# kdexd/probnmn-clevr

Hardware: AMD Instinct MI355X
Metric: CLEVR questions/sec (joint_training step) (higher is better)
Workload: dtype f32; 1 GPU; joint_training_ours.yml (NMN + seq2seq + REINFORCE), global batch 1024 = 1024 questions per GPU x 1 (BASELINE configs[3]), 14x14x1024 features, half of the batch with program supervision, fwd+bwd+[all-reduce]+clamp+Adam; global_batch=1024, per_gpu_batch=1024, parallelism=dp1

## Files before the change

include/probnmn_hip.h:

```cpp
#ifndef PROBNMN_HIP_H
#define PROBNMN_HIP_H

#include <stdint.h>

#ifdef __cplusplus
extern "C" {
#endif

#define PNMN_EINVAL (-1)
#define PNMN_ESHAPE (-2)

#define PNMN_CHANNELS 128

typedef struct pnmn_conv_item {
    const float* in;
    const float* in2;
    const float* mask;
    const float* gate;
    const float* weight;
    const float* bias;
    float*       out;
    int32_t      dilation;
    int32_t      flags;
    const float* mb_feats;
// ... 356 lines not shown
    const int64_t* tokens;
    int64_t        token_stride;
    const float*   w_hh;
    const float*   w_ih;
    const float*   bias;
    float*         hs;
    float*         cs;
    float*         act;
    const float*   dhs;
    float*         dgates;
    int32_t        B, T, dep, reserved;
} pnmn_lstm_stack_job;
int64_t pnmn_lstm_stack_workspace_bytes(const pnmn_lstm_stack_job* jobs , int n, int backward);
int pnmn_lstm_stack_fwd(const pnmn_lstm_stack_job* jobs , int n, void* workspace, void* stream);
int pnmn_lstm_stack_bwd(const pnmn_lstm_stack_job* jobs , int n, void* workspace, void* stream);

typedef struct pnmn_lstm_dropout_desc {
    float*   hsd;
    uint64_t seed;
    int64_t  row_offset;
    float    p;
    int32_t  reserved;
} pnmn_lstm_dropout_desc;
int pnmn_lstm_dropout(const float* x, float* y, int rows, int T, int H, float p, uint64_t seed, int64_t row_offset, void* stream);
int pnmn_lstm_stack_fwd_dropout(const pnmn_lstm_stack_job* jobs , const pnmn_lstm_dropout_desc* drops , int n,
                                void* workspace, void* stream);
int pnmn_lstm_stack_bwd_dropout(const pnmn_lstm_stack_job* jobs , const pnmn_lstm_dropout_desc* drops , int n,
                                void* workspace, void* stream);

#define PNMN_GEMM_MAX 8
#define PNMN_GEMM_A_TRANSPOSED 1
#define PNMN_GEMM_B_TRANSPOSED 2
#define PNMN_GEMM_ACCUMULATE   4
typedef struct pnmn_gemm_desc {
    const float* a;
    const float* b;
    float*       c;
    const float* bias;
    int64_t      lda, ldb, ldc;
    int32_t      M, N, K;
    int32_t      flags;
    int32_t      split_k;
    int32_t      shift_t;
    const float* shift_h0;
    int64_t      ld_h0;
    float*       workspace;
    float*       colsum;
    float*       colsum2;
} pnmn_gemm_desc;
int pnmn_gemm(const pnmn_gemm_desc* descs , int n, void* stream);
int pnmn_gemm_cus(const pnmn_gemm_desc* descs , int n, int max_workgroups, void* stream);
int64_t pnmn_gemm_workspace_bytes(int M, int N, int split_k);
int pnmn_gemm_split_k(int M, int N, int K, int cus);

int pnmn_colsum(const float* x, int64_t ld, int R, int C, float* out, float* out2, int accumulate, void* workspace, void* stream);
int64_t pnmn_colsum_workspace_bytes(int R, int C);

int pnmn_abi_version(void);

#ifdef __cplusplus
}
#endif
#endif
```

probnmn-clevr_amd/csrc/gemm.hip:

```cpp
#include <hip/hip_runtime.h>
#include <stdint.h>

#include <type_traits>

#include "../../include/probnmn_hip.h"
#include "global_ptr.h"
#include "lds_optin.h"

namespace {

typedef float f32x16 __attribute__((ext_vector_type(16)));
using pnmn::as_global;
using pnmn::gfloat;

constexpr int TM = 128, TN = 128, TK = 32;
constexpr int OP_FLOATS = TM * TK;
using lchar = __attribute__((address_space(3))) char;
using gchar = __attribute__((address_space(1))) char;

struct Batch {
    pnmn_gemm_desc d[PNMN_GEMM_MAX];
    int first[PNMN_GEMM_MAX + 1];
    int n;
};

template <bool KC>
__device__ __forceinline__ void load_tile(const gfloat* base, int64_t ld, int row0, int k0, int rows, int K, bool vec, int tid,
                                          f32x4 (&r)[4], int shift_t, const gfloat* h0, int64_t ld_h0) {
#pragma unroll
    for (int j = 0; j < 4; ++j) {
        const int p = tid + 256 * j;
        f32x4 v = f32x4{0.f, 0.f, 0.f, 0.f};
        if (KC) {
            const int row = row0 + (p >> 3), k = k0 + 4 * (p & 7);
            if (row < rows && k < K) {
                const gfloat* src = base + (int64_t)row * ld + k;
                if (vec && k + 3 < K) {
                    v = pnmn::load4(src);
                } else {
#pragma unroll
                    for (int e = 0; e < 4; ++e)
                        if (k + e < K) v[e] = src[e];
                }
            }
        } else {
            const int k = k0 + (p >> 5), row = row0 + 4 * (p & 31);
            if (k < K && row < rows) {
                const gfloat* src;
                bool zero = false;
                if (shift_t > 0) {
                    const int b = k / shift_t;
// ... 64 lines not shown
    int64_t piece, step;
    uint32_t off;

    __device__ __forceinline__ void start(const gfloat* origin, int64_t ld, int row0, int k0, int tid) {
        const int wave = __builtin_amdgcn_readfirstlane(tid >> 6), lane = tid & 63;
        const uint64_t o64 = (uint64_t)(uintptr_t)origin;
        const gchar* o = (const gchar*)(((uint64_t)(uint32_t)__builtin_amdgcn_readfirstlane((int)(o64 >> 32)) << 32) |
                                        (uint32_t)__builtin_amdgcn_readfirstlane((int)(uint32_t)o64));
        if (KC) {
            const int c = (lane & 7) ^ (lane >> 4);
            base = o + ((int64_t)(row0 + 32 * wave) * ld + k0) * 4;
            v0 = (uint32_t)((lane >> 3) * ld) * 4u + 16u * c, v1 = (uint32_t)((lane >> 3) * ld) * 4u + 16u * (c ^ 4);
            piece = 32 * ld, step = 4 * TK, off = (uint32_t)wave * 32u * 128u;
        } else {
            base = o + ((int64_t)(k0 + 8 * wave) * ld + row0) * 4;
            v0 = v1 = (uint32_t)((lane >> 5) * ld) * 4u + 16u * (lane & 31);
            piece = 8 * ld, step = 4 * (int64_t)TK * ld, off = (uint32_t)wave * 8u * 512u;
        }
    }
    __device__ __forceinline__ void issue(float* tile) {
        const uint32_t dst = __builtin_amdgcn_readfirstlane((uint32_t)(uintptr_t)((lchar*)tile)) + off;
#pragma unroll
        for (int j = 0; j < 4; ++j) {
            const uint64_t src = (uint64_t)(uintptr_t)(base + j * piece);
            asm volatile("s_mov_b32 m0, %2\n\ts_nop 0\n\tglobal_load_lds_dwordx4 %0, %1"
                         :
                         : "v"(KC && (j & 1) ? v1 : v0), "s"(src), "s"(dst + 1024u * j)
                         : "memory");
        }
        base += step;
    }
};

template <bool AKC, bool BKC>
__device__ __forceinline__ void contract(const pnmn_gemm_desc& d, int m0, int n0, int kbeg, int kend, float* lds, f32x16 (&acc)[2][2],
                                         bool want_cs, float (&cs)[2]) {
    const int tid = threadIdx.x, wave = tid >> 6, lane = tid & 63, i = lane & 31, h = lane >> 5;
    const int wm = wave >> 1, wn = wave & 1;
    const gfloat* A = as_global(d.a);
    const gfloat* Bm = as_global(d.b);
    const gfloat* h0 = as_global(d.shift_h0);
    const bool avec = (d.lda & 3) == 0 && ((uintptr_t)d.a & 15) == 0;
    const bool bvec = (d.ldb & 3) == 0 && ((uintptr_t)d.b & 15) == 0 && (d.shift_t == 0 || d.shift_h0 == nullptr ||
                                                                       ((d.ld_h0 & 3) == 0 && ((uintptr_t)d.shift_h0 & 15) == 0));
    float* la = lds;
    float* lb = lds + 2 * OP_FLOATS;
    const bool adir = avec && m0 + TM <= d.M, bdir = bvec && n0 + TN <= d.N && (BKC || d.shift_t == 0);
    const int kfull = kbeg + (kend - kbeg) / TK * TK;
    const float rcp_t = d.shift_t > 0 ? 1.f / (float)d.shift_t : 0.f;
    Direct<AKC> da;
    Direct<BKC> db;
    da.start(A, d.lda, m0, kbeg, tid);
    db.start(Bm, d.ldb, n0, kbeg, tid);
    auto loop = [&](auto ad_tag, auto bd_tag, int lo, int hi) {
        constexpr bool AD = decltype(ad_tag)::value, BD = decltype(bd_tag)::value;
        f32x4 ra[4], rb[4];
        auto fetch = [&](int k0, int st) {
            if constexpr (AD)
                da.issue(la + st * OP_FLOATS);
            else
                load_tile<AKC>(A, d.lda, m0, k0, d.M, kend, avec, tid, ra, 0, nullptr, 0);
            if constexpr (BD)
                db.issue(lb + st * OP_FLOATS);
            else if constexpr (AD && !BKC)
                load_tile_shift(Bm, d.ldb, n0, k0, tid, rb, d.shift_t, rcp_t, h0, d.ld_h0);
            else
                load_tile<BKC>(Bm, d.ldb, n0, k0, d.N, kend, bvec, tid, rb, BKC ? 0 : d.shift_t, h0, d.ld_h0);
        };
        auto commit = [&](int st) {
            if constexpr (!AD) store_tile<AKC>(la + st * OP_FLOATS, tid, ra);
            if constexpr (!BD) store_tile<BKC>(lb + st * OP_FLOATS, tid, rb);
        };
        if (lo >= hi) return;
        fetch(lo, 0);
        commit(0);
        asm volatile("s_waitcnt vmcnt(0)" ::: "memory");
        __syncthreads();
        int cur = 0;
        for (int k0 = lo; k0 < hi; k0 += TK) {
            const bool more = k0 + TK < hi;
            if (more) fetch(k0 + TK, cur ^ 1);
            const float* ca = la + cur * OP_FLOATS;
            const float* cb = lb + cur * OP_FLOATS;
#pragma unroll
            for (int q = 0; q < 4; ++q) {
                f32x4 a[2], b[2];
#pragma unroll
                for (int t = 0; t < 2; ++t) {
                    a[t] = frag<AKC>(ca, 64 * wm + 32 * t + i, q, h);
                    b[t] = frag<BKC>(cb, 64 * wn + 32 * t + i, q, h);
                }
                if (!AKC && want_cs) {
#pragma unroll
                    for (int t = 0; t < 2; ++t) cs[t] += (a[t][0] + a[t][1]) + (a[t][2] + a[t][3]);
                }
#pragma unroll
                for (int s = 0; s < 4; ++s)
#pragma unroll
                    for (int mt = 0; mt < 2; ++mt)
#pragma unroll
                        for (int nt = 0; nt < 2; ++nt)
                            acc[mt][nt] = __builtin_amdgcn_mfma_f32_32x32x2f32(a[mt][s], b[nt][s], acc[mt][nt], 0, 0, 0);
            }
            if (more) commit(cur ^ 1);
            asm volatile("s_waitcnt vmcnt(0)" ::: "memory");
            __syncthreads();
            cur ^= 1;
        }
    };
    using yes = std::true_type;
    using no = std::false_type;
    if (adir && bdir) {
        loop(yes{}, yes{}, kbeg, kfull);
        loop(no{}, no{}, kfull, kend);
    } else if (!BKC && adir && bvec && d.shift_t > 0 && n0 + TN <= d.N && kend <= (1 << 21)) {
        if constexpr (!BKC) {
            loop(yes{}, no{}, kbeg, kfull);
            loop(no{}, no{}, kfull, kend);
        }
    } else {
        loop(no{}, no{}, kbeg, kend);
    }
}

__global__ __launch_bounds__(256) __attribute__((amdgpu_waves_per_eu(2, 2))) void gemm_kernel(const Batch batch) {
    extern __shared__ __attribute__((aligned(16))) float lds[];
    for (int unit = blockIdx.x; unit < batch.first[batch.n]; unit += gridDim.x) {
    int pi = 0;
    while (pi + 1 < batch.n && unit >= batch.first[pi + 1]) ++pi;
    const pnmn_gemm_desc d = batch.d[pi];
    const int local = unit - batch.first[pi];
    const int tiles_n = (d.N + TN - 1) / TN, tiles_m = (d.M + TM - 1) / TM;
    const int split = d.split_k > 1 ? d.split_k : 1;
    const int chunk = local % split, tile = local / split;
    const int tm = tile / tiles_n, tn = tile % tiles_n;
    const int m0 = tm * TM, n0 = tn * TN;
    const int ktiles = (d.K + TK - 1) / TK;
    const int per = ktiles / split, extra = ktiles % split;
    const int kt0 = chunk * per + (chunk < extra ? chunk : extra);
    const int kt1 = kt0 + per + (chunk < extra ? 1 : 0);
    const int kbeg = kt0 * TK, kend = kt1 * TK < d.K ? kt1 * TK : d.K;

    f32x16 acc[2][2];
#pragma unroll
    for (int mt = 0; mt < 2; ++mt)
#pragma unroll
        for (int nt = 0; nt < 2; ++nt)
#pragma unroll
            for (int r = 0; r < 16; ++r) acc[mt][nt][r] = 0.f;
    const bool akc = !(d.flags & PNMN_GEMM_A_TRANSPOSED), bkc = (d.flags & PNMN_GEMM_B_TRANSPOSED) != 0;
    const bool want_cs = d.colsum != nullptr && !akc && tn == 0 && ((threadIdx.x >> 6) & 1) == 0;
    const bool tile_cs = d.colsum != nullptr && !akc && tn == 0;
    float cs[2] = {0.f, 0.f};
    if (kbeg < kend) {
        if (akc && bkc)
            contract<true, true>(d, m0, n0, kbeg, kend, lds, acc, false, cs);
        else if (akc)
            contract<true, false>(d, m0, n0, kbeg, kend, lds, acc, false, cs);
        else if (bkc)
            contract<false, true>(d, m0, n0, kbeg, kend, lds, acc, want_cs, cs);
        else
            contract<false, false>(d, m0, n0, kbeg, kend, lds, acc, want_cs, cs);
    }

    int tid = threadIdx.x, m0e = m0, n0e = n0;
    asm volatile("" : "+v"(tid), "+s"(m0e), "+s"(n0e));
    const int wave = tid >> 6, lane = tid & 63, i = lane & 31, h = lane >> 5;
    const int wm = wave >> 1, wn = wave & 1;
    if (tile_cs) {
        if (want_cs) {
#pragma unroll
            for (int t = 0; t < 2; ++t) lds[h * TM + 64 * wm + 32 * t + i] = cs[t];
        }
        __syncthreads();
        if (tid < TM) {
            const float t = lds[tid] + lds[TM + tid];
            if (split > 1) {
                as_global(d.workspace)[(size_t)tiles_m * tiles_n * split * (TM * TN) + ((size_t)tm * split + chunk) * TM + tid] = t;
            } else if (m0e + tid < d.M) {
                d.colsum[m0e + tid] = t;
                if (d.colsum2) d.colsum2[m0e + tid] = t;
            }
        }
        __syncthreads();
    }
    if (split > 1) {
        gfloat* ws = as_global(d.workspace) + ((size_t)tile * split + chunk) * (TM * TN);
#pragma unroll
        for (int mt = 0; mt < 2; ++mt)
#pragma unroll
            for (int nt = 0; nt < 2; ++nt)
#pragma unroll
                for (int r = 0; r < 16; ++r)
                    ws[(64 * wm + 32 * mt + 8 * (r >> 2) + 4 * h + (r & 3)) * TN + 64 * wn + 32 * nt + i] = acc[mt][nt][r];
        continue;
    }
    gfloat* C = as_global(d.c);
    const gfloat* bias = as_global(d.bias);
    const bool accumulate = (d.flags & PNMN_GEMM_ACCUMULATE) != 0;
#pragma unroll
    for (int nt = 0; nt < 2; ++nt) {
        const int col = n0e + 64 * wn + 32 * nt + i;
        if (col >= d.N) continue;
        const float bv = d.bias ? bias[col] : 0.f;
#pragma unroll
        for (int mt = 0; mt < 2; ++mt)
#pragma unroll
            for (int r = 0; r < 16; ++r) {
                const int row = m0e + 64 * wm + 32 * mt + 8 * (r >> 2) + 4 * h + (r & 3);
                if (row < d.M) {
                    gfloat* dst = C + (int64_t)row * d.ldc + col;
                    float v = acc[mt][nt][r] + bv;
                    if (accumulate) v += *dst;
                    *dst = v;
                }
            }
    }
    }
}

__global__ __launch_bounds__(256) void gemm_reduce_kernel(const Batch batch) {
    int pi = 0;
    while (pi + 1 < batch.n && (int)blockIdx.x >= batch.first[pi + 1]) ++pi;
    const pnmn_gemm_desc d = batch.d[pi];
    const int local = blockIdx.x - batch.first[pi];
    const int tiles_n = (d.N + TN - 1) / TN;
    const int quarter = local & 3, tile = local >> 2;
    const int m0 = (tile / tiles_n) * TM + 32 * quarter, n0 = (tile % tiles_n) * TN;
    const int split = d.split_k, tid = threadIdx.x;
    const gfloat* wt = as_global(d.workspace) + (size_t)tile * split * (TM * TN) + quarter * (32 * TN);
    f32x4 sum[4];
#pragma unroll
    for (int j = 0; j < 4; ++j) sum[j] = f32x4{0.f, 0.f, 0.f, 0.f};
    for (int c = 0; c < split; ++c) {
        const gfloat* wc = wt + (size_t)c * (TM * TN);
        f32x4 v[4];
#pragma unroll
        for (int j = 0; j < 4; ++j) v[j] = pnmn::load4(wc + 4 * (tid + 256 * j));
#pragma unroll
        for (int j = 0; j < 4; ++j) sum[j] += v[j];
    }
    if (d.colsum && (d.flags & PNMN_GEMM_A_TRANSPOSED) && quarter == 0 && tile % tiles_n == 0 && tid < TM) {
        const int tiles_m = (d.M + TM - 1) / TM, tm = tile / tiles_n;
        const gfloat* wc = as_global(d.workspace) + (size_t)tiles_m * tiles_n * split * (TM * TN) + (size_t)tm * split * TM + tid;
        float t = 0.f;
        for (int c = 0; c < split; ++c) t += wc[(size_t)c * TM];
        if (tm * TM + tid < d.M) {
            d.colsum[tm * TM + tid] = t;
            if (d.colsum2) d.colsum2[tm * TM + tid] = t;
        }
    }
    gfloat* C = as_global(d.c);
    const gfloat* bias = as_global(d.bias);
    const bool accumulate = (d.flags & PNMN_GEMM_ACCUMULATE) != 0;
    const bool cvec = (d.ldc & 3) == 0 && ((uintptr_t)d.c & 15) == 0;
#pragma unroll
    for (int j = 0; j < 4; ++j) {
        const int p = tid + 256 * j, row = m0 + (p >> 5), col = n0 + 4 * (p & 31);
        if (row >= d.M || col >= d.N) continue;
        gfloat* dst = C + (int64_t)row * d.ldc + col;
        f32x4 v = sum[j];
        if (cvec && col + 3 < d.N) {
            if (d.bias) {
// ... 53 lines not shown
        last_flag = old == slices - 1;
        if (last_flag) counter[blockIdx.x] = 0;
    }
    __syncthreads();
    if (!last_flag || c >= C) return;
    __threadfence();
    float total = 0.f;
    for (int k = 0; k < slices; ++k) total += __builtin_nontemporal_load(partial + (size_t)k * C + c);
    if (accumulate) total += out[c];
    out[c] = total;
    if (out2) out2[c] = total;
}

}

extern "C" int64_t pnmn_gemm_workspace_bytes(int M, int N, int split_k) {
    if (split_k <= 1) return 0;
    const int64_t tiles_m = (M + TM - 1) / TM, tiles = tiles_m * ((N + TN - 1) / TN);
    return (tiles * split_k * (TM * TN) + tiles_m * split_k * TM) * (int64_t)sizeof(float);
}

extern "C" int pnmn_gemm_split_k(int M, int N, int K, int cus) {
    const int64_t tiles = (int64_t)((M + TM - 1) / TM) * ((N + TN - 1) / TN);
    const int ktiles = (K + TK - 1) / TK;
    if (cus <= 0) cus = 256;
    int64_t want = (2 * (int64_t)cus + tiles - 1) / tiles;
    if (tiles >= cus) want = 1;
    const int most = ktiles / 4 > 0 ? ktiles / 4 : 1;
    if (want > most) want = most;
    if (want > 64) want = 64;
    return want < 1 ? 1 : (int)want;
}

extern "C" int pnmn_gemm(const pnmn_gemm_desc* descs, int n, void* stream) { return pnmn_gemm_cus(descs, n, 0, stream); }

extern "C" int pnmn_gemm_cus(const pnmn_gemm_desc* descs, int n, int max_workgroups, void* stream) {
    if (n <= 0) return 0;
    if (!descs || n > PNMN_GEMM_MAX) return PNMN_EINVAL;
    Batch b;
    int blocks = 0, live = 0;
    for (int k = 0; k < n; ++k) {
        const pnmn_gemm_desc& d = descs[k];
        if (d.M <= 0 || d.N <= 0) continue;
        if (!d.a || !d.b || !d.c || d.K < 0) return PNMN_EINVAL;
        if (d.split_k > 1 && !d.workspace) return PNMN_EINVAL;
        if (d.shift_t > 0 && (d.flags & PNMN_GEMM_B_TRANSPOSED)) return PNMN_ESHAPE;
        if (d.colsum && !(d.flags & PNMN_GEMM_A_TRANSPOSED)) return PNMN_ESHAPE;
        b.d[live] = d;
        b.first[live] = blocks;
        const int tiles = ((d.M + TM - 1) / TM) * ((d.N + TN - 1) / TN);
        blocks += tiles * (d.split_k > 1 ? d.split_k : 1);
        ++live;
    }
    if (!live) return 0;
    b.first[live] = blocks;
    b.n = live;
    constexpr size_t lds = (size_t)4 * OP_FLOATS * sizeof(float);
    static std::atomic<uint64_t> cfg{0};
    if (const int e = pnmn::opt_in_lds(reinterpret_cast<const void*>(gemm_kernel), lds, cfg)) return e;
    const int grid = (max_workgroups > 0 && max_workgroups < blocks) ? max_workgroups : blocks;
    hipLaunchKernelGGL(gemm_kernel, dim3(grid), dim3(256), lds, static_cast<hipStream_t>(stream), b);
    Batch r;
    int rblocks = 0, rlive = 0;
    for (int k = 0; k < live; ++k) {
        if (b.d[k].split_k <= 1) continue;
        r.d[rlive] = b.d[k];
        r.first[rlive] = rblocks;
        rblocks += 4 * ((b.d[k].M + TM - 1) / TM) * ((b.d[k].N + TN - 1) / TN);
        ++rlive;
    }
    if (rlive) {
        r.first[rlive] = rblocks;
        r.n = rlive;
        hipLaunchKernelGGL(gemm_reduce_kernel, dim3(rblocks), dim3(256), 0, static_cast<hipStream_t>(stream), r);
    }
    return (int)hipGetLastError();
}

extern "C" int64_t pnmn_colsum_workspace_bytes(int R, int C) {
    (void)R;
    return (int64_t)128 * C * sizeof(float) + (int64_t)((C + 255) / 256) * sizeof(int);
}

extern "C" int pnmn_colsum(const float* x, int64_t ld, int R, int C, float* out, float* out2, int accumulate, void* workspace,
                           void* stream) {
    if (C <= 0) return 0;
    if (!out || !workspace || (R > 0 && !x)) return PNMN_EINVAL;
    int slices = (R + 63) / 64;
    if (slices > 128) slices = 128;
    if (slices < 1) slices = 1;
    float* partial = static_cast<float*>(workspace);
    int* counter = reinterpret_cast<int*>(partial + (size_t)128 * C);
    const int vec = (ld & 3) == 0 && ((uintptr_t)x & 15) == 0;
    hipLaunchKernelGGL(colsum_kernel, dim3((C + 255) / 256, slices), dim3(256), 0, static_cast<hipStream_t>(stream), x, ld, R, C,
                       partial, counter, out, out2, accumulate, vec);
    return (int)hipGetLastError();
}
```

probnmn-clevr_amd/probnmn/_hip.py:

```python
import ctypes
import os
import time
from typing import Dict, Optional

import numpy as np
import torch

_HERE = os.path.dirname(os.path.abspath(__file__))
LIB_PATH = os.environ.get("PNMN_LIB") or os.path.join(os.path.dirname(_HERE), "lib", "libprobnmn_hip.so")

CHANNELS = 128
CONV_ACCUMULATE = 1
CONV_ATOMIC = 2
CONV_MASKBWD = 4
CONV_DATTN = 16


class HipLibraryError(RuntimeError):
    pass


_lib: Optional[ctypes.CDLL] = None

_P = ctypes.c_void_p
# ... 51 lines not shown
    "pnmn_attn_lstm_fwd": (_P,) * 15 + (_I,) * 9 + (ctypes.c_uint64, ctypes.c_uint64, _P, ctypes.c_int64, _P),
    "pnmn_attn_lstm_bwd": (_P,) * 14 + (_I,) * 4 + (_P,),
    "pnmn_attn_lstm_group_workspace_bytes": (_P, _I, _I),
    "pnmn_attn_lstm_fwd_group": (_P, _I, _I, _P, _P),
    "pnmn_attn_lstm_bwd_group": (_P, _I, _I, _P, _P),
    "pnmn_attn_denc": (_P, _P, _P, _P, _P, _P, _I, _I, _I, _I, _P),
    "pnmn_conv_nhwc_launches": (_I, _I, _I, _I, _I, _I),
    "pnmn_conv_force_split": (_I,),
    "pnmn_run_launches": (_P, _I, _P),
    "pnmn_conv2d_nhwc": (_P, _P),
    "pnmn_conv2d_weight_floats": (_I, _I, _I, _I),
    "pnmn_maxpool3x3s2_nhwc": (_P, _P, _I, _I, _I, _I, _P),
    "pnmn_launch_trace_begin": (),
    "pnmn_launch_trace_end": (_P, _I, _P),
    "pnmn_set_rows": (_P, _I, _P),
    "pnmn_trunk_planner_create": (_P, _P),
    "pnmn_trunk_planner_destroy": (_P,),
    "pnmn_trunk_plan_and_launch": (_P, _P, _P),
    "pnmn_trunk_last_forward": (_P, _P, _I),
    "pnmn_trunk_last_records_bytes": (_P, _P, ctypes.c_int64),
    "pnmn_plan_batch": (_P, _P, ctypes.c_int64, _P, _P, _I),
    "pnmn_compile_programs": (_P, _I, _I, _P, _I, _I, _P, _P, _P, _P),
    "pnmn_sample_tokens": (_P, _P, _P, _I, _I, _I, ctypes.c_uint64, ctypes.c_uint64, ctypes.c_uint32, _I, _I, _I, _P),
    "pnmn_lstm_stack_workspace_bytes": (_P, _I, _I),
    "pnmn_lstm_stack_fwd": (_P, _I, _P, _P),
    "pnmn_lstm_stack_bwd": (_P, _I, _P, _P),
    "pnmn_lstm_dropout": (_P, _P, _I, _I, _I, _F, ctypes.c_uint64, ctypes.c_int64, _P),
    "pnmn_lstm_stack_fwd_dropout": (_P, _P, _I, _P, _P),
    "pnmn_lstm_stack_bwd_dropout": (_P, _P, _I, _P, _P),
    "pnmn_gemm": (_P, _I, _P),
    "pnmn_gemm_cus": (_P, _I, _I, _P),
    "pnmn_gemm_workspace_bytes": (_I, _I, _I),
    "pnmn_gemm_split_k": (_I, _I, _I, _I),
    "pnmn_colsum": (_P, ctypes.c_int64, _I, _I, _P, _P, _I, _P, _P),
    "pnmn_colsum_workspace_bytes": (_I, _I),
}


ABI_VERSION = 13


def lib() -> ctypes.CDLL:
    global _lib
    if _lib is None:
        if not os.path.exists(LIB_PATH):
            raise HipLibraryError(
                "libprobnmn_hip.so not found at %s -- build it with `python -c 'import "
                "__graft_entry__ as g; g.build()'` (hipcc --offload-arch=gfx950); there is no "
                "fallback path" % LIB_PATH
            )
        handle = ctypes.CDLL(LIB_PATH)
        for name, argtypes in SIGNATURES.items():
            fn = getattr(handle, name)
            fn.restype = ctypes.c_int64 if name.endswith("_bytes") else ctypes.c_int
            fn.argtypes = list(argtypes)
        if handle.pnmn_abi_version() != ABI_VERSION:
            raise HipLibraryError("%s has ABI version %d, this package binds version %d -- rebuild the library"
                                  % (LIB_PATH, handle.pnmn_abi_version(), ABI_VERSION))
        _lib = handle
    return _lib


_TRACE = None


def check(code: int, what: str) -> None:
# ... 71 lines not shown
     ("a_channels", _i32), ("b_channels", _i32), ("is_max", _i32), ("reserved", _i32)]
)
MASKBWD_ITEM = np.dtype([("dx", _u64), ("feats", _u64), ("attn", _u64), ("dfeats", _u64), ("dattn", _u64)])
AXPY_ITEM = np.dtype([("src", _u64), ("dst", _u64), ("n", np.int64)])
DERIVE_JOB = np.dtype([("src", _u64), ("src2", _u64), ("dst", _u64), ("n", _i32), ("k", _i32), ("ld", _i32), ("kind", _i32)])
PLAN_IN = np.dtype([(n, _u64) for n in ("tables", "nprims", "tids", "examples", "base", "tokens", "w3", "b3", "wt3",
                                         "dotw", "dotb", "params", "grads", "wt", "act", "gact", "feat", "gfeat",
                                         "final_", "gfinal", "ones")]
                   + [(n, _i32) for n in ("n_templates", "pmax", "nv", "cmax", "hw", "channels", "wgrad_chunk",
                                          "wgrad_groups", "fuse_mask_bwd", "sole_writer", "sort_by_weight", "reserved")])
TRUNK_CONFIG = np.dtype([(n, _u64) for n in ("kinds", "w3", "b3", "wt3", "dotw", "dotb")]
                        + [(n, _i32) for n in ("n_kinds", "channels", "H", "W", "wgrad_chunk", "wgrad_groups", "fuse_mask_bwd",
                                               "sole_writer", "sort_by_weight", "reserved")])
TRUNK_IO = np.dtype([(n, _u64) for n in ("programs", "params", "grads", "wt", "act", "gact", "feat", "gfeat", "final_", "gfinal",
                                          "ones")]
                    + [("act_capacity", np.int64)]
                    + [(n, _u64) for n in ("fwd_tail", "bwd_head", "bwd_tail", "bwd", "valid")]
                    + [("arena_floats", np.int64)]
                    + [(n, _i32) for n in ("n_programs", "length", "n_fwd_tail", "n_bwd_head", "n_bwd_tail", "bwd_capacity",
                                           "need_backward", "launch", "n_bwd", "bwd_piece_cut", "n_prims", "n_fwd", "depth",
                                           "n_invalid", "n_feat_result", "conv_cus", "wgrad_cus", "n_conv", "n_proj", "reserved")]
                    + [("touched_tokens", _u64, (4,))])
DECODER_FWD_JOB = np.dtype([(n, _u64) for n in ("xe", "etable", "enc", "mask", "h0", "w_c", "w_hh", "w_p", "b_p", "hs", "cs", "act",
                                                  "ctx", "probs", "tokens", "in_tokens")]
                           + [("in_token_stride", np.int64), ("seed", _u64), ("row_offset", _u64)]
                           + [(n, _i32) for n in ("B", "T", "S", "V", "sample", "pad_index", "unk_index", "start_index")])
DECODER_BWD_JOB = np.dtype([(n, _u64) for n in ("dhs", "act", "cs", "hs", "probs", "enc", "mask", "h0", "w_c_t", "w_hh_t", "dgates",
                                                  "dctx", "dscore", "weights", "dh0")]
                           + [(n, _i32) for n in ("B", "T", "S", "reserved")])
GEMM_DESC = np.dtype([(n, _u64) for n in ("a", "b", "c", "bias")] + [(n, np.int64) for n in ("lda", "ldb", "ldc")]
                     + [(n, _i32) for n in ("M", "N", "K", "flags", "split_k", "shift_t")]
                     + [("shift_h0", _u64), ("ld_h0", np.int64), ("workspace", _u64), ("colsum", _u64), ("colsum2", _u64)])
GEMM_MAX, GEMM_A_T, GEMM_B_T, GEMM_ACC = 8, 1, 2, 4
LSTM_STACK_JOB = np.dtype([("xp", _u64), ("tokens", _u64), ("token_stride", np.int64)] + [(n, _u64) for n in ("w_hh", "w_ih", "bias", "hs", "cs", "act", "dhs", "dgates")]
                          + [(n, _i32) for n in ("B", "T", "dep", "reserved")])
LSTM_STACK_JOBS = 6
LSTM_DROPOUT_DESC = np.dtype([("hsd", _u64), ("seed", _u64), ("row_offset", np.int64), ("p", np.float32), ("reserved", _i32)])
TOKEN_SEG = np.dtype([("src", _u64), ("index", _u64), ("row_stride", np.int64), ("rows", _i32), ("width", _i32)])
EINVAL, ESHAPE, EAGAIN = -1, -2, -3
ADAM_ITEM = np.dtype([("param", _u64), ("grad", _u64), ("exp_avg", _u64), ("exp_avg_sq", _u64), ("n", np.int64),
                      ("bc1", np.float32), ("bc2_sqrt", np.float32)])

LAUNCH = np.dtype([("a", _u64), ("b", _u64), ("c", _u64), ("op", _i32), ("n", _i32), ("p", _i32, (8,))])
CONV2D_DESC = np.dtype([("x", _u64), ("w", _u64), ("scale", _u64), ("shift", _u64), ("residual", _u64), ("y", _u64),
                        ("N", _i32), ("H", _i32), ("W", _i32), ("Cin", _i32), ("Ho", _i32), ("Wo", _i32), ("Cout", _i32),
                        ("kh", _i32), ("kw", _i32), ("stride", _i32), ("pad", _i32), ("relu", _i32)])
LAUNCH_TIMING = np.dtype([("op", _i32), ("n", _i32), ("p", _i32, (8,)), ("n_items", _i32), ("ms", np.float32),
                          ("flops", np.float64), ("bytes", np.float64)])
(OP_CONV, OP_WGRAD, OP_TRANSPOSE_WEIGHTS, OP_DOT_FWD, OP_DOT_BWD, OP_SAME_FWD, OP_SAME_BWD, OP_MINMAX_FWD, OP_MINMAX_BWD,
 OP_MASK_BWD, OP_MAXPOOL_FWD, OP_MAXPOOL_BWD, OP_NCHW_TO_NHWC, OP_SET_ROWS, OP_ACCUMULATE, OP_ZERO, OP_FEAT_GATHER) = range(17)


class LaunchList:

    def __init__(self):
        self._rows = []

    def add(self, op: int, n: int, a: int, b: int = 0, c: int = 0, p=()) -> None:
        q = tuple(p) + (0,) * (8 - len(p))
        self._rows.append((a, b, c, op | (n << 32), q[0] | (q[1] << 32), q[2] | (q[3] << 32), q[4] | (q[5] << 32),
                           q[6] | (q[7] << 32)))

    def __len__(self) -> int:
        return len(self._rows)

    def run(self, stream: int, what: str) -> None:
# ... 135 lines not shown
```

probnmn-clevr_amd/probnmn/runtime/seq_plan.py:

```python
from typing import Dict, List, Optional

import numpy as np
import torch

from probnmn import _hip


SPLIT_SLOTS = int(__import__("os").environ.get("PNMN_PLAN_SPLIT_SLOTS", "512"))
SPLIT_MIN_KTILES = int(__import__("os").environ.get("PNMN_PLAN_SPLIT_MIN", "8"))
USE_STACK = True
import os as _os
STACK_FWD_ENCODERS = int(_os.environ.get("PNMN_PLAN_FWD_ENC", "2"))
STACK_PG_ENCODER = int(_os.environ.get("PNMN_PLAN_PG_ENC", "1"))
STACK_BWD_ENCODERS = int(_os.environ.get("PNMN_PLAN_BWD_ENC", "0"))
DECODER_BWD_GROUP = int(_os.environ.get("PNMN_PLAN_DEC_GROUP", "3"))
GEMM_WORKGROUPS = int(_os.environ.get("PNMN_PLAN_GEMM_WGS", "0"))
USE_AUX_STREAM = _os.environ.get("PNMN_PLAN_AUX", "0") != "0"
_AUX_STREAMS: Dict = {}


def _aux_stream(dev: torch.device) -> "torch.cuda.Stream":
    key = dev.index if dev.index is not None else torch.cuda.current_device()
    if key not in _AUX_STREAMS:
        _AUX_STREAMS[key] = torch.cuda.Stream(device=dev)
    return _AUX_STREAMS[key]


class PlanUnsupported(Exception):
    """The models / shapes are outside what the plan is built for: the trainer keeps the eager passes."""


class _Calls(list):
    def add(self, name: str, *args) -> None:
        self.append((getattr(_hip.lib(), name), args, name))

    def add_fn(self, name: str, fn) -> None:
        self.append((fn, (), name))

    def run(self) -> None:
        for fn, args, name in self:
            rc = fn(*args)
            if rc:
# ... 60 lines not shown
        self.with_prior = with_prior
        B = n + m
        self.B = B
        D = pg._max_decoding_steps
        self.D = D
        if _hip.decoder_workspace_bytes([n, m], False) <= 0 or _hip.decoder_workspace_bytes([B], False) <= 0 \
                or int(lib.pnmn_lstm_seq_workspace_bytes(B, 0)) <= 0:
            raise PlanUnsupported("batch does not fit the multi-CU recurrent kernels in one launch")
        self._bufs: Dict[str, torch.Tensor] = {}
        self._keep: List = []
        self.anchor = torch.zeros((), device=dev, requires_grad=True)
        self.fwd_pg_enc, self.fwd_pg, self.fwd_qr, self.fwd_prior, self.bwd = _Calls(), _Calls(), _Calls(), _Calls(), _Calls()
        self._derived_sig = None
        self._build()

    def buf(self, name: str, *shape, dtype=torch.float32, zero: bool = False) -> torch.Tensor:
        if name in self._bufs:
            raise KeyError(name)
        t = (torch.zeros if zero else torch.empty)(*shape, dtype=dtype, device=self.dev)
        self._bufs[name] = t
        return t

    def bytes_buf(self, name: str, nbytes: int, zero: bool = False) -> torch.Tensor:
        return self.buf(name, max(int(nbytes), 16), dtype=torch.uint8, zero=zero)

    def __getitem__(self, name: str) -> torch.Tensor:
        return self._bufs[name]

    def _gemm(self, calls: _Calls, name: str, descs) -> None:
        lib = _hip.lib()
        for lo in range(0, len(descs), _hip.GEMM_MAX):
            part = descs[lo:lo + _hip.GEMM_MAX]
            rec = np.zeros(len(part), _hip.GEMM_DESC)
            tiles = [((d["M"] + 127) // 128) * ((d["N"] + 127) // 128) for d in part]
            ktiles = [(d["K"] + 31) // 32 for d in part]
            auto = [i for i, d in enumerate(part) if d.get("split") == "auto"]
            fixed_units = sum(t for i, t in enumerate(tiles) if i not in auto)
            chunk_len, best = SPLIT_MIN_KTILES, None
            for cand in range(SPLIT_MIN_KTILES, 129):
                splits = [max(1, min(-(-ktiles[i] // cand), 64)) for i in auto]
                units = fixed_units + sum(tiles[i] * sp for i, sp in zip(auto, splits))
                longest = max([-(-ktiles[i] // sp) for i, sp in zip(auto, splits)] + [ktiles[i] for i in range(len(part)) if i not in auto] + [1])
                rounds = units // SPLIT_SLOTS + (0.6 if units % SPLIT_SLOTS else 0.0)
                cost = rounds * longest + 4.0 * sum(tiles[i] * sp for i, sp in zip(auto, splits) if sp > 1) / SPLIT_SLOTS
                if best is None or cost < best:
                    chunk_len, best = cand, cost
            for i, d in enumerate(part):
                r = rec[i]
                r["a"], r["b"], r["c"] = d["a"], d["b"], d["c"]
                r["lda"], r["ldb"], r["ldc"] = d["lda"], d["ldb"], d["ldc"]
                r["M"], r["N"], r["K"] = d["M"], d["N"], d["K"]
                r["flags"] = (_hip.GEMM_A_T if d.get("ta") else 0) | (_hip.GEMM_B_T if d.get("tb") else 0) | (_hip.GEMM_ACC if d.get("acc") else 0)
                r["bias"] = d.get("bias", 0)
                split = d.get("split", 1)
                if split == "auto":
                    split = max(1, min(-(-ktiles[i] // chunk_len), 64))
                r["split_k"] = split
                if split > 1:
                    ws = self.bytes_buf("%s.ws%d" % (name, lo + i), lib.pnmn_gemm_workspace_bytes(d["M"], d["N"], split), zero=True)
                    r["workspace"] = ws.data_ptr()
                r["shift_t"], r["shift_h0"], r["ld_h0"] = d.get("shift_t", 0), d.get("h0", 0), d.get("ld_h0", 0)
                r["colsum"], r["colsum2"] = d.get("colsum", 0), d.get("colsum2", 0)
            self._keep.append(rec)
            calls.add("pnmn_gemm_cus", rec.ctypes.data, len(rec), GEMM_WORKGROUPS, self.stream)

    def _encoder_prepare(self, calls: _Calls, tag: str, mm: Optional[_Model], derived, tokens: torch.Tensor, width: int, rows: int,
                         drop_first: bool, emb: torch.Tensor, pad_idx, lstm, want_last: bool = True, p: float = 0.0) -> Dict:
        st = self.stream
        model = mm.model if mm is not None else self.prior
        pad, bos, eos = model._pad_index, model._start_index, model._end_index
        T = width + 2 - int(drop_first)
        V = emb.size(0)
        f = self.buf
        e = dict(tag=tag, mm=mm, derived=derived, lstm=lstm, T=T, rows=rows, V=V, pad_idx=-1 if pad_idx is None else pad_idx, emb=emb,
                 want_last=want_last,
                 src=f(tag + ".src", rows, T, dtype=torch.long), fmask=f(tag + ".fmask", rows, T), last=f(tag + ".last", rows, dtype=torch.int32),
                 table=f(tag + ".table", V, 1024), hs1=f(tag + ".hs1", rows, T, 256), cs1=f(tag + ".cs1", rows, T, 256),
                 act1=f(tag + ".act1", rows, T, 1024), hs2=f(tag + ".hs2", rows, T, 256), cs2=f(tag + ".cs2", rows, T, 256),
                 act2=f(tag + ".act2", rows, T, 1024), p=p, seed=0, row_offset=0, drop_recs=[])
        if p > 0:
            e["hsd"] = f(tag + ".hsd", rows, T, 256)
        calls.add("pnmn_token_prep", tokens.data_ptr(), tokens.stride(0), rows, width, pad, bos, eos, int(drop_first), e["src"].data_ptr(),
                  e["fmask"].data_ptr(), e["last"].data_ptr(), st)
        calls.add("pnmn_token_table_fwd", emb.data_ptr(), lstm.weight_ih_l0.data_ptr(), lstm.weight_ih_l0.stride(0),
                  derived["l0.b"].data_ptr(), V, 256, 1024, e["table"].data_ptr(), st)
        if want_last:
            e["enc"], e["h"] = f(tag + ".enc", rows, T, 256), f(tag + ".h", rows, 256)
        return e

    def _stack_jobs(self, encs: List[Dict], backward: bool) -> np.ndarray:
        jobs = np.zeros(2 * len(encs), _hip.LSTM_STACK_JOB)
        for k, e in enumerate(encs):
            d = e["derived"]
            if not backward:
                a, b = jobs[2 * k], jobs[2 * k + 1]
# ... 460 lines not shown
```

Before: 37220 questions/s.

## Move split-K planning to C, add partial-tail splitting and direct shifted B loads

Moves the split-K chunk-length search from Python into a C planner (pnmn_gemm_plan). The planner adds a new mode: when the last GEMM leaves a partial final round of workgroups, only those leftover tiles are split along K while the rest stay whole. This aims to fill the idle slots of the last wave. It also adds a DirectShift loader that streams the time-shifted B operand straight into LDS with global_load_lds, replacing the register-staged path, so shifted LSTM-style GEMMs can use direct LDS loads. The extra encoding in flags and the negative split_k add complexity and reduction overhead, and the cost heuristics may mis-predict.

```diff
diff --git a/include/probnmn_hip.h b/include/probnmn_hip.h
--- a/include/probnmn_hip.h
+++ b/include/probnmn_hip.h
@@ -412,6 +412,9 @@
 #define PNMN_GEMM_A_TRANSPOSED 1
 #define PNMN_GEMM_B_TRANSPOSED 2
 #define PNMN_GEMM_ACCUMULATE   4
+#define PNMN_GEMM_SPLIT_AUTO   8
+#define PNMN_GEMM_SHIFT_REGISTERS 16
+#define PNMN_GEMM_WHOLE_SHIFT  8
 typedef struct pnmn_gemm_desc {
     const float* a;
     const float* b;
@@ -432,6 +435,9 @@
 int pnmn_gemm_cus(const pnmn_gemm_desc* descs , int n, int max_workgroups, void* stream);
 int64_t pnmn_gemm_workspace_bytes(int M, int N, int split_k);
 int pnmn_gemm_split_k(int M, int N, int K, int cus);
+int pnmn_gemm_plan(pnmn_gemm_desc* descs , int n, int cus);
+int64_t pnmn_gemm_plan_workspace_bytes(const pnmn_gemm_desc* desc);
+int pnmn_gemm_plan_units(const pnmn_gemm_desc* desc);
 
 int pnmn_colsum(const float* x, int64_t ld, int R, int C, float* out, float* out2, int accumulate, void* workspace, void* stream);
 int64_t pnmn_colsum_workspace_bytes(int R, int C);
diff --git a/probnmn-clevr_amd/csrc/gemm.hip b/probnmn-clevr_amd/csrc/gemm.hip
--- a/probnmn-clevr_amd/csrc/gemm.hip
+++ b/probnmn-clevr_amd/csrc/gemm.hip
@@ -17,6 +17,16 @@
 constexpr int OP_FLOATS = TM * TK;
 using lchar = __attribute__((address_space(3))) char;
 using gchar = __attribute__((address_space(1))) char;
+
+__host__ __device__ inline int plan_chunks(const pnmn_gemm_desc& d) { return d.split_k > 1 ? d.split_k : d.split_k < -1 ? -d.split_k : 1; }
+__host__ __device__ inline int plan_whole(const pnmn_gemm_desc& d) {
+    return d.split_k < -1 ? (int)((uint32_t)d.flags >> PNMN_GEMM_WHOLE_SHIFT) : 0;
+}
+__host__ __device__ inline int desc_tiles(const pnmn_gemm_desc& d) { return ((d.M + TM - 1) / TM) * ((d.N + TN - 1) / TN); }
+__host__ __device__ inline int plan_units(const pnmn_gemm_desc& d) {
+    const int tiles = desc_tiles(d), whole = plan_whole(d);
+    return whole + (tiles - whole) * plan_chunks(d);
+}
 
 struct Batch {
     pnmn_gemm_desc d[PNMN_GEMM_MAX];
@@ -147,6 +157,38 @@
     }
 };
 
+__device__ __attribute__((aligned(16))) const float zero_row[TN] = {};
+
+struct DirectShift {
+    const gchar* base;
+    const gchar* init;
+    int64_t ld, ld_init;
+    int k, shift_t;
+    float rcp_t;
+    uint32_t off;
+
+    __device__ __forceinline__ void start(const gfloat* origin, int64_t ldb, int col0, int k0, int tid, int t, float rcp, const gfloat* h0,
+                                          int64_t ld_h0) {
+        const int wave = __builtin_amdgcn_readfirstlane(tid >> 6), lane = tid & 63;
+        base = (const gchar*)origin + 4 * (int64_t)(col0 + 4 * (lane & 31));
+        init = h0 ? (const gchar*)h0 + 4 * (int64_t)(col0 + 4 * (lane & 31)) : (const gchar*)as_global(zero_row) + 16 * (lane & 31);
+        ld = 4 * ldb, ld_init = h0 ? 4 * ld_h0 : 0;
+        k = k0 + 8 * wave + (lane >> 5), shift_t = t, rcp_t = rcp;
+        off = (uint32_t)wave * 8u * 512u;
+    }
+    __device__ __forceinline__ void issue(float* tile) {
+        const uint32_t dst = __builtin_amdgcn_readfirstlane((uint32_t)(uintptr_t)((lchar*)tile)) + off;
+#pragma unroll
+        for (int j = 0; j < 4; ++j) {
+            const int r = k + 2 * j;
+            const int b = (int)(((float)r + 0.5f) * rcp_t);
+            const gchar* src = r == b * shift_t ? init + (int64_t)b * ld_init : base + (int64_t)(r - 1) * ld;
+            asm volatile("s_mov_b32 m0, %1\n\ts_nop 0\n\tglobal_load_lds_dwordx4 %0, off" : : "v"(src), "s"(dst + 1024u * j) : "memory");
+        }
+        k += TK;
+    }
+};
+
 template <bool AKC, bool BKC>
 __device__ __forceinline__ void contract(const pnmn_gemm_desc& d, int m0, int n0, int kbeg, int kend, float* lds, f32x16 (&acc)[2][2],
                                          bool want_cs, float (&cs)[2]) {
@@ -161,22 +203,28 @@
     float* la = lds;
     float* lb = lds + 2 * OP_FLOATS;
     const bool adir = avec && m0 + TM <= d.M, bdir = bvec && n0 + TN <= d.N && (BKC || d.shift_t == 0);
+    const bool shift_direct = (d.flags & PNMN_GEMM_SHIFT_REGISTERS) == 0;
     const int kfull = kbeg + (kend - kbeg) / TK * TK;
     const float rcp_t = d.shift_t > 0 ? 1.f / (float)d.shift_t : 0.f;
     Direct<AKC> da;
     Direct<BKC> db;
+    DirectShift ds;
     da.start(A, d.lda, m0, kbeg, tid);
     db.start(Bm, d.ldb, n0, kbeg, tid);
+    if constexpr (!BKC) ds.start(Bm, d.ldb, n0, kbeg, tid, d.shift_t, rcp_t, h0, d.ld_h0);
     auto loop = [&](auto ad_tag, auto bd_tag, int lo, int hi) {
-        constexpr bool AD = decltype(ad_tag)::value, BD = decltype(bd_tag)::value;
+        constexpr bool AD = decltype(ad_tag)::value;
+        constexpr int BD = decltype(bd_tag)::value;
         f32x4 ra[4], rb[4];
         auto fetch = [&](int k0, int st) {
             if constexpr (AD)
                 da.issue(la + st * OP_FLOATS);
             else
                 load_tile<AKC>(A, d.lda, m0, k0, d.M, kend, avec, tid, ra, 0, nullptr, 0);
-            if constexpr (BD)
+            if constexpr (BD == 1)
                 db.issue(lb + st * OP_FLOATS);
+            else if constexpr (BD == 2)
+                ds.issue(lb + st * OP_FLOATS);
             else if constexpr (AD && !BKC)
                 load_tile_shift(Bm, d.ldb, n0, k0, tid, rb, d.shift_t, rcp_t, h0, d.ld_h0);
             else
@@ -225,12 +273,16 @@
     };
     using yes = std::true_type;
     using no = std::false_type;
+    using shifted = std::integral_constant<int, 2>;
     if (adir && bdir) {
         loop(yes{}, yes{}, kbeg, kfull);
         loop(no{}, no{}, kfull, kend);
     } else if (!BKC && adir && bvec && d.shift_t > 0 && n0 + TN <= d.N && kend <= (1 << 21)) {
         if constexpr (!BKC) {
-            loop(yes{}, no{}, kbeg, kfull);
+            if (shift_direct)
+                loop(yes{}, shifted{}, kbeg, kfull);
+            else
+                loop(yes{}, no{}, kbeg, kfull);
             loop(no{}, no{}, kfull, kend);
         }
     } else {
@@ -246,8 +298,11 @@
     const pnmn_gemm_desc d = batch.d[pi];
     const int local = unit - batch.first[pi];
     const int tiles_n = (d.N + TN - 1) / TN, tiles_m = (d.M + TM - 1) / TM;
-    const int split = d.split_k > 1 ? d.split_k : 1;
-    const int chunk = local % split, tile = local / split;
+    const int chunks = plan_chunks(d), whole = plan_whole(d);
+    const bool cut = chunks > 1 && local >= whole;
+    const int split = cut ? chunks : 1;
+    const int chunk = cut ? (local - whole) % chunks : 0, wtile = cut ? (local - whole) / chunks : 0;
+    const int tile = cut ? whole + wtile : local;
     const int tm = tile / tiles_n, tn = tile % tiles_n;
     const int m0 = tm * TM, n0 = tn * TN;
     const int ktiles = (d.K + TK - 1) / TK;
@@ -300,7 +355,7 @@
         __syncthreads();
     }
     if (split > 1) {
-        gfloat* ws = as_global(d.workspace) + ((size_t)tile * split + chunk) * (TM * TN);
+        gfloat* ws = as_global(d.workspace) + ((size_t)wtile * split + chunk) * (TM * TN);
 #pragma unroll
         for (int mt = 0; mt < 2; ++mt)
 #pragma unroll
@@ -340,10 +395,11 @@
     const pnmn_gemm_desc d = batch.d[pi];
     const int local = blockIdx.x - batch.first[pi];
     const int tiles_n = (d.N + TN - 1) / TN;
-    const int quarter = local & 3, tile = local >> 2;
+    const int whole = plan_whole(d);
+    const int quarter = local & 3, tile = whole + (local >> 2);
     const int m0 = (tile / tiles_n) * TM + 32 * quarter, n0 = (tile % tiles_n) * TN;
-    const int split = d.split_k, tid = threadIdx.x;
-    const gfloat* wt = as_global(d.workspace) + (size_t)tile * split * (TM * TN) + quarter * (32 * TN);
+    const int split = plan_chunks(d), tid = threadIdx.x;
+    const gfloat* wt = as_global(d.workspace) + (size_t)(tile - whole) * split * (TM * TN) + quarter * (32 * TN);
     f32x4 sum[4];
 #pragma unroll
     for (int j = 0; j < 4; ++j) sum[j] = f32x4{0.f, 0.f, 0.f, 0.f};
@@ -463,6 +519,95 @@
     return want < 1 ? 1 : (int)want;
 }
 
+constexpr int SPLIT_MIN_KTILES = 8, SPLIT_MAX_KTILES = 128, SPLIT_MAX_CHUNKS = 64;
+constexpr double STARTED_ROUND = 0.6, PARTIAL_KTILES = 4.0, LONE_ROUND = 0.9, REDUCE_LAUNCH_KTILES = 2.0;
+
+extern "C" int pnmn_gemm_plan(pnmn_gemm_desc* descs, int n, int cus) {
+    if (n <= 0) return 0;
+    if (!descs || n > PNMN_GEMM_MAX) return PNMN_EINVAL;
+    if (cus <= 0) cus = 256;
+    const int64_t slots = 2 * (int64_t)cus;
+    int64_t tiles[PNMN_GEMM_MAX], fixed_units = 0;
+    int ktiles[PNMN_GEMM_MAX], longest_fixed = 1, last = -1;
+    bool aut[PNMN_GEMM_MAX], any = false;
+    for (int i = 0; i < n; ++i) {
+        pnmn_gemm_desc& d = descs[i];
+        const bool live = d.M > 0 && d.N > 0;
+        aut[i] = live && (d.flags & PNMN_GEMM_SPLIT_AUTO) != 0;
+        if (aut[i]) d.split_k = 1, d.flags &= (1 << PNMN_GEMM_WHOLE_SHIFT) - 1;
+        tiles[i] = live ? desc_tiles(d) : 0;
+        ktiles[i] = (d.K + TK - 1) / TK;
+        if (!live) continue;
+        last = i;
+        any |= aut[i];
+        if (!aut[i]) {
+            fixed_units += plan_units(d);
+            const int len = (ktiles[i] + plan_chunks(d) - 1) / plan_chunks(d);
+            if (len > longest_fixed) longest_fixed = len;
+        }
+    }
+    if (!any) return 0;
+    auto chunks_at = [&](int i, int len) {
+        int sp = (ktiles[i] + len - 1) / len;
+        if (sp > SPLIT_MAX_CHUNKS) sp = SPLIT_MAX_CHUNKS;
+        if (sp > ktiles[i] / SPLIT_MIN_KTILES) sp = ktiles[i] / SPLIT_MIN_KTILES;
+        return sp < 1 ? 1 : sp;
+    };
+    int chunk_len = SPLIT_MIN_KTILES;
+    double best = -1.0;
+    for (int cand = SPLIT_MIN_KTILES; cand <= SPLIT_MAX_KTILES; ++cand) {
+        int64_t units = fixed_units, partials = 0;
+        int longest = longest_fixed;
+        for (int i = 0; i < n; ++i) {
+            if (!aut[i]) continue;
+            const int sp = chunks_at(i, cand), len = (ktiles[i] + sp - 1) / sp;
+            units += tiles[i] * sp;
+            if (sp > 1) partials += tiles[i] * sp;
+            if (len > longest) longest = len;
+        }
+        const double rounds = (double)(units / slots) + (units % slots ? STARTED_ROUND : 0.0);
+        const double cost = rounds * longest + PARTIAL_KTILES * (double)partials / (double)slots;
+        if (best < 0.0 || cost < best) chunk_len = cand, best = cost;
+    }
+    int64_t units = fixed_units;
+    for (int i = 0; i < n; ++i) {
+        if (!aut[i]) continue;
+        descs[i].split_k = chunks_at(i, chunk_len);
+        units += tiles[i] * descs[i].split_k;
+    }
+    pnmn_gemm_desc& t = descs[last];
+    const int64_t rest = units % slots;
+    if (aut[last] && t.split_k == 1 && !t.colsum && units > slots && rest > 0 && rest <= tiles[last] &&
+        tiles[last] - rest < ((int64_t)1 << (31 - PNMN_GEMM_WHOLE_SHIFT))) {
+        int most = (int)(slots / rest);
+        if (most > ktiles[last] / SPLIT_MIN_KTILES) most = ktiles[last] / SPLIT_MIN_KTILES;
+        if (most > SPLIT_MAX_CHUNKS) most = SPLIT_MAX_CHUNKS;
+        int chunks = 1;
+        double least = (2 * rest <= slots ? LONE_ROUND : 1.0) * ktiles[last];
+        for (int c = 2; c <= most; ++c) {
+            const double cost = (ktiles[last] + c - 1) / c + PARTIAL_KTILES * (double)(rest * c) / (double)slots + REDUCE_LAUNCH_KTILES;
+            if (cost < least) chunks = c, least = cost;
+        }
+        if (chunks > 1) {
+            t.split_k = -chunks;
+            t.flags |= (int32_t)((tiles[last] - rest) << PNMN_GEMM_WHOLE_SHIFT);
+        }
+    }
+    return 0;
+}
+
+extern "C" int pnmn_gemm_plan_units(const pnmn_gemm_desc* desc) {
+    if (!desc || desc->M <= 0 || desc->N <= 0) return 0;
+    return plan_units(*desc);
+}
+
+extern "C" int64_t pnmn_gemm_plan_workspace_bytes(const pnmn_gemm_desc* desc) {
+    if (!desc || desc->M <= 0 || desc->N <= 0) return 0;
+    if (desc->split_k < -1)
+        return (int64_t)(desc_tiles(*desc) - plan_whole(*desc)) * plan_chunks(*desc) * (TM * TN) * (int64_t)sizeof(float);
+    return pnmn_gemm_workspace_bytes(desc->M, desc->N, desc->split_k);
+}
+
 extern "C" int pnmn_gemm(const pnmn_gemm_desc* descs, int n, void* stream) { return pnmn_gemm_cus(descs, n, 0, stream); }
 
 extern "C" int pnmn_gemm_cus(const pnmn_gemm_desc* descs, int n, int max_workgroups, void* stream) {
@@ -474,13 +619,13 @@
         const pnmn_gemm_desc& d = descs[k];
         if (d.M <= 0 || d.N <= 0) continue;
         if (!d.a || !d.b || !d.c || d.K < 0) return PNMN_EINVAL;
-        if (d.split_k > 1 && !d.workspace) return PNMN_EINVAL;
+        if ((d.split_k > 1 || d.split_k < -1) && !d.workspace) return PNMN_EINVAL;
+        if (d.split_k < -1 && (plan_whole(d) >= desc_tiles(d) || d.colsum)) return PNMN_ESHAPE;
         if (d.shift_t > 0 && (d.flags & PNMN_GEMM_B_TRANSPOSED)) return PNMN_ESHAPE;
         if (d.colsum && !(d.flags & PNMN_GEMM_A_TRANSPOSED)) return PNMN_ESHAPE;
         b.d[live] = d;
         b.first[live] = blocks;
-        const int tiles = ((d.M + TM - 1) / TM) * ((d.N + TN - 1) / TN);
-        blocks += tiles * (d.split_k > 1 ? d.split_k : 1);
+        blocks += plan_units(d);
         ++live;
     }
     if (!live) return 0;
@@ -494,10 +639,10 @@
     Batch r;
     int rblocks = 0, rlive = 0;
     for (int k = 0; k < live; ++k) {
-        if (b.d[k].split_k <= 1) continue;
+        if (plan_chunks(b.d[k]) <= 1) continue;
         r.d[rlive] = b.d[k];
         r.first[rlive] = rblocks;
-        rblocks += 4 * ((b.d[k].M + TM - 1) / TM) * ((b.d[k].N + TN - 1) / TN);
+        rblocks += 4 * (desc_tiles(b.d[k]) - plan_whole(b.d[k]));
         ++rlive;
     }
     if (rlive) {
diff --git a/probnmn-clevr_amd/probnmn/_hip.py b/probnmn-clevr_amd/probnmn/_hip.py
--- a/probnmn-clevr_amd/probnmn/_hip.py
+++ b/probnmn-clevr_amd/probnmn/_hip.py
@@ -107,6 +107,9 @@
     "pnmn_gemm_cus": (_P, _I, _I, _P),
     "pnmn_gemm_workspace_bytes": (_I, _I, _I),
     "pnmn_gemm_split_k": (_I, _I, _I, _I),
+    "pnmn_gemm_plan": (_P, _I, _I),
+    "pnmn_gemm_plan_workspace_bytes": (_P,),
+    "pnmn_gemm_plan_units": (_P,),
     "pnmn_colsum": (_P, ctypes.c_int64, _I, _I, _P, _P, _I, _P, _P),
     "pnmn_colsum_workspace_bytes": (_I, _I),
 }
@@ -244,6 +247,7 @@
                      + [(n, _i32) for n in ("M", "N", "K", "flags", "split_k", "shift_t")]
                      + [("shift_h0", _u64), ("ld_h0", np.int64), ("workspace", _u64), ("colsum", _u64), ("colsum2", _u64)])
 GEMM_MAX, GEMM_A_T, GEMM_B_T, GEMM_ACC = 8, 1, 2, 4
+GEMM_SPLIT_AUTO, GEMM_SHIFT_REGISTERS, GEMM_WHOLE_SHIFT = 8, 16, 8
 LSTM_STACK_JOB = np.dtype([("xp", _u64), ("tokens", _u64), ("token_stride", np.int64)] + [(n, _u64) for n in ("w_hh", "w_ih", "bias", "hs", "cs", "act", "dhs", "dgates")]
                           + [(n, _i32) for n in ("B", "T", "dep", "reserved")])
 LSTM_STACK_JOBS = 6
diff --git a/probnmn-clevr_amd/probnmn/runtime/seq_plan.py b/probnmn-clevr_amd/probnmn/runtime/seq_plan.py
--- a/probnmn-clevr_amd/probnmn/runtime/seq_plan.py
+++ b/probnmn-clevr_amd/probnmn/runtime/seq_plan.py
@@ -6,8 +6,7 @@
 from probnmn import _hip
 
 
-SPLIT_SLOTS = int(__import__("os").environ.get("PNMN_PLAN_SPLIT_SLOTS", "512"))
-SPLIT_MIN_KTILES = int(__import__("os").environ.get("PNMN_PLAN_SPLIT_MIN", "8"))
+SPLIT_CUS = int(__import__("os").environ.get("PNMN_PLAN_SPLIT_CUS", "256"))
 USE_STACK = True
 import os as _os
 STACK_FWD_ENCODERS = int(_os.environ.get("PNMN_PLAN_FWD_ENC", "2"))
@@ -134,19 +133,6 @@
         for lo in range(0, len(descs), _hip.GEMM_MAX):
             part = descs[lo:lo + _hip.GEMM_MAX]
             rec = np.zeros(len(part), _hip.GEMM_DESC)
-            tiles = [((d["M"] + 127) // 128) * ((d["N"] + 127) // 128) for d in part]
-            ktiles = [(d["K"] + 31) // 32 for d in part]
-            auto = [i for i, d in enumerate(part) if d.get("split") == "auto"]
-            fixed_units = sum(t for i, t in enumerate(tiles) if i not in auto)
-            chunk_len, best = SPLIT_MIN_KTILES, None
-            for cand in range(SPLIT_MIN_KTILES, 129):
-                splits = [max(1, min(-(-ktiles[i] // cand), 64)) for i in auto]
-                units = fixed_units + sum(tiles[i] * sp for i, sp in zip(auto, splits))
-                longest = max([-(-ktiles[i] // sp) for i, sp in zip(auto, splits)] + [ktiles[i] for i in range(len(part)) if i not in auto] + [1])
-                rounds = units // SPLIT_SLOTS + (0.6 if units % SPLIT_SLOTS else 0.0)
-                cost = rounds * longest + 4.0 * sum(tiles[i] * sp for i, sp in zip(auto, splits) if sp > 1) / SPLIT_SLOTS
-                if best is None or cost < best:
-                    chunk_len, best = cand, cost
             for i, d in enumerate(part):
                 r = rec[i]
                 r["a"], r["b"], r["c"] = d["a"], d["b"], d["c"]
@@ -156,13 +142,16 @@
                 r["bias"] = d.get("bias", 0)
                 split = d.get("split", 1)
                 if split == "auto":
-                    split = max(1, min(-(-ktiles[i] // chunk_len), 64))
+                    r["flags"] |= _hip.GEMM_SPLIT_AUTO
+                    split = 1
                 r["split_k"] = split
-                if split > 1:
-                    ws = self.bytes_buf("%s.ws%d" % (name, lo + i), lib.pnmn_gemm_workspace_bytes(d["M"], d["N"], split), zero=True)
-                    r["workspace"] = ws.data_ptr()
                 r["shift_t"], r["shift_h0"], r["ld_h0"] = d.get("shift_t", 0), d.get("h0", 0), d.get("ld_h0", 0)
                 r["colsum"], r["colsum2"] = d.get("colsum", 0), d.get("colsum2", 0)
+            _hip.check(lib.pnmn_gemm_plan(rec.ctypes.data, len(rec), SPLIT_CUS), "pnmn_gemm_plan")
+            for i in range(len(part)):
+                nbytes = int(lib.pnmn_gemm_plan_workspace_bytes(rec.ctypes.data + i * rec.itemsize))
+                if nbytes > 0:
+                    rec[i]["workspace"] = self.bytes_buf("%s.ws%d" % (name, lo + i), nbytes, zero=True).data_ptr()
             self._keep.append(rec)
             calls.add("pnmn_gemm_cus", rec.ctypes.data, len(rec), GEMM_WORKGROUPS, self.stream)
 
```

Result: no change. 37480 questions/s, median of 5 (+0.7%).
